# heathsc/bs_call

Measured on AMD Instinct MI355X. Metric: genome positions called/sec, higher is better.
Workload: dtype f64

## Files before the change

bs_call_amd/csrc/prepdev.hip:

```cpp
#include <hip/hip_runtime.h>
#include <stdint.h>

#include "../../include/bscall_amd.h"

#define FLT_QUAL 63u

struct bsc_prep_plan {
  uint64_t src;
  uint64_t ms;
  uint32_t rl0;
  uint32_t w0, wl;
  uint32_t nm;
  uint32_t mark_l, mark_r;
  uint32_t out_len;
  uint32_t present;
  uint32_t trim_l, trim_r;
};

struct bsc_prep_desc {
  uint64_t srcw;
  uint32_t pk;
  int32_t pc;
};
#define PD_PRESENT 1u
#define PD_EDITED 2u
#define PD_SLOW 8u

#define PREP_CNT_WORDS 8u
#define PREP_CNT_SLOTS 64u
#define PE_ORI 1u
#define PE_READ 2u
#define PE_LIST 4u
#define PE_SOFT_POS 6u
#define PE_SOFT_ILL 7u
#define PE_INDEL 8u
#define PE_CAP 9u
#define PE_PROF_CAP 10u
#define PE_PROF_RANGE 11u

struct prep_rd {
  uint32_t w0, wl;
};
__device__ static __forceinline__ void d_left_trim(prep_rd &r, uint32_t l) {
  if (l > 0) {
    if (l >= r.wl) r.wl = 0;
    else {
      r.w0 += l;
      r.wl -= l;
    }
  }
}
__device__ static __forceinline__ void d_right_trim(prep_rd &r, uint32_t l) {
  if (l > 0) {
    if (l >= r.wl) r.wl = 0;
    else r.wl -= l;
  }
}

__device__ static __forceinline__ uint32_t d_qual(const uint8_t *sp, uint32_t i, uint32_t rl0, uint32_t mark_l, uint32_t mark_r) {
  return (i < mark_l || i >= rl0 - mark_r) ? FLT_QUAL : (uint32_t)sp[i] >> 2;
}

__device__ static __forceinline__ uint32_t d_ld32(const uint8_t *p);
__device__ static uint32_t d_mean_qual(const uint8_t *sp, const prep_rd &r, uint32_t rl0, uint32_t mark_l, uint32_t mark_r) {
  const uint32_t lo = r.w0 > mark_l ? r.w0 : mark_l;
  const uint32_t e0 = r.w0 + r.wl, e1 = rl0 - mark_r;
  const uint32_t hi = e0 < e1 ? e0 : e1;
  uint32_t tot = 0, n = 0, i = lo;
#define MQ_DWORD(w_)                                                                                                                   \
  {                                                                                                                                    \
    const uint32_t q = ((w_) >> 2) & 0x3f3f3f3fu;                                                                                      \
    const uint32_t nz = ((q ^ 0x3f3f3f3fu) + 0x7f7f7f7fu) & 0x80808080u;  \
    n += (uint32_t)__popc(nz);                                                                                                         \
    tot = __builtin_amdgcn_sad_u8(q & ((nz >> 7) * 0xffu), 0u, tot);                                       \
  }
  for (; i + 16u <= hi; i += 16u) {
    uint4 v;
    __builtin_memcpy(&v, sp + i, 16);
    MQ_DWORD(v.x) MQ_DWORD(v.y) MQ_DWORD(v.z) MQ_DWORD(v.w)
  }
  for (; i + 4u <= hi; i += 4u) MQ_DWORD(d_ld32(sp + i))
#undef MQ_DWORD
  for (; i < hi; i++) {
    const uint32_t q = (uint32_t)sp[i] >> 2;
    if (q != FLT_QUAL) {
      tot += q;
      n++;
    }
  }
  return n > 0 ? tot / n : 0;
}

__global__ __launch_bounds__(256) void bsc_prep_plan_kernel(const bsc_raw_template *__restrict__ raw, uint32_t nr, const uint8_t *__restrict__ seq,
                                                            uint64_t seq_bytes, const bsc_misms *__restrict__ misms_in, uint64_t n_misms_in,
                                                            bsc_prep_params par, bsc_misms *__restrict__ ms_work,
                                                            bsc_prep_plan *__restrict__ plan, bsc_prep_desc *__restrict__ desc,
                                                            unsigned long long *__restrict__ out_len,
                                                            bsc_template *__restrict__ tpl_out, unsigned long long *__restrict__ cnt,
                                                            uint32_t *__restrict__ max_pos1) {
  const uint32_t ti = blockIdx.x * 256u + threadIdx.x;
  unsigned long long n_clip = 0, n_overlap = 0;
  uint32_t err = 0;
  if (ti < nr) {
    const bsc_raw_template t = raw[ti];
    bsc_prep_plan P[2];
    prep_rd rd[2];
    uint32_t nm[2];
    bsc_misms *ms[2];
    bool edited[2] = {false, false};
    uint32_t pos[2] = {t.pos[0], t.pos[1]};
    if (t.orientation > 1) err = PE_ORI;
#pragma unroll
    for (int k = 0; k < 2 && !err; k++) {
      if (t.len[k] && (t.off[k] > seq_bytes || t.len[k] > seq_bytes - t.off[k])) err = PE_READ + (uint32_t)k;
      else if (t.n_misms[k] && (t.misms_off[k] > n_misms_in || t.n_misms[k] > n_misms_in - t.misms_off[k])) err = PE_LIST + (uint32_t)k;
    }
    if (!err) {
      const int msk = t.orientation == 0 ? 0 : 1;
#pragma unroll
      for (int k = 0; k < 2; k++) {
        const int side = k ^ msk;
        const uint32_t rl = t.len[k];
        const int32_t lt = side ? par.left_trim[1] : par.left_trim[0], rt = side ? par.right_trim[1] : par.right_trim[0];
        P[k].src = t.off[k];
        P[k].ms = t.misms_off[k];
        P[k].rl0 = rl;
        P[k].mark_l = lt > 0 ? ((uint32_t)lt < rl ? (uint32_t)lt : rl) : 0u;
        P[k].mark_r = rt > 0 ? ((uint32_t)rt < rl ? (uint32_t)rt : rl) : 0u;
        P[k].present = rl != 0;
        P[k].trim_l = P[k].trim_r = 0;
        rd[k].w0 = 0;
        rd[k].wl = rl;
        nm[k] = t.n_misms[k];
        ms[k] = ms_work + t.misms_off[k];
        for (uint32_t z = 0; z < nm[k]; z++) ms[k][z] = misms_in[t.misms_off[k] + z];
      }
#pragma unroll
      for (int k = 0; k < 2 && !err; k++) {
        const uint32_t rl = rd[k].wl;
        if (rl == 0) continue;
        int nclip = 0;
        uint32_t adj = 0;
        const uint32_t n0 = nm[k];
        for (uint32_t z = 0; z < n0; z++) {
          bsc_misms *m = ms[k] + z;
          if (m->type == BSC_MISMS_SOFT) {
            if (z && z != n0 - 1) { err = PE_SOFT_POS; break; }
            nclip++;
            if (!m->position) {
              if (m->size >= rl) { err = PE_SOFT_ILL; break; }
              adj = m->size;
              n_clip += adj;
              P[k].trim_l = adj;
              d_left_trim(rd[k], adj);
            } else {
              if (m->position + m->size != rl) { err = PE_SOFT_ILL; break; }
              d_right_trim(rd[k], m->size);
              P[k].trim_r = m->size;
              n_clip += m->size;
            }
          } else if (nclip) {
            m->position -= adj;
            ms[k][z - (uint32_t)nclip] = *m;
          }
        }
        if (nclip) nm[k] -= (uint32_t)nclip;
      }
    }
    if (!err) {
      const uint32_t rdl[2] = {rd[0].wl, rd[1].wl};
      if (rdl[0] > 0 && rdl[1] > 0) {
        int rev;
        int32_t overlap;
        if (pos[0] <= pos[1]) {
          overlap = (int32_t)(t.reference_span[0] - pos[1] + pos[0]);
          rev = 0;
        } else {
          overlap = (int32_t)(t.reference_span[1] + pos[1] - pos[0]);
          rev = 1;
        }
        if (pos[0] + t.reference_span[0] >= pos[1]) {
          int tr;
          if (t.reference_span[0] > t.reference_span[1]) tr = 1;
          else if (t.reference_span[0] < t.reference_span[1]) tr = 0;
          else
            tr = d_mean_qual(seq + P[0].src, rd[0], P[0].rl0, P[0].mark_l, P[0].mark_r) <=
                         d_mean_qual(seq + P[1].src, rd[1], P[1].rl0, P[1].mark_l, P[1].mark_r)
                     ? 0
                     : 1;
          const int right = (rev && tr) || !(rev || tr);
          if (!right) {
            if (tr) pos[1] += (uint32_t)overlap;
            else pos[0] += (uint32_t)overlap;
          }
          bsc_misms *mm = tr ? ms[1] : ms[0];
          prep_rd rdt = tr ? rd[1] : rd[0];
          const uint32_t rdl_t = tr ? rdl[1] : rdl[0], span_t = tr ? t.reference_span[1] : t.reference_span[0];
          uint32_t num = tr ? nm[1] : nm[0];
          if (!num) {
            if (right) d_right_trim(rdt, (uint32_t)overlap);
            else d_left_trim(rdt, (uint32_t)overlap);
          } else {
            int trimmed = 0;
            if (right) {
              const uint32_t xx = span_t - (uint32_t)overlap;
              int64_t adj = 0;
              for (uint32_t z = 0; z < num; z++) {
                bsc_misms *m = mm + z;
                if ((int64_t)m->position + adj >= (int64_t)xx) {
                  const int64_t trim = (int64_t)rdl_t - xx + adj;
                  d_right_trim(rdt, (uint32_t)trim);
                  num = z;
                  trimmed = 1;
                  break;
                }
                if (m->type == BSC_MISMS_INS) {
                  if ((int64_t)m->position + adj + m->size >= (int64_t)xx) {
                    const int64_t trim = (int64_t)rdl_t - m->position;
                    m->size = (uint32_t)((int64_t)xx - ((int64_t)m->position + adj));
                    d_right_trim(rdt, (uint32_t)trim);
                    num = z + 1;
                    trimmed = 1;
                  }
                  adj += m->size;
                } else if (m->type == BSC_MISMS_DEL) adj -= m->size;
              }
              if (!trimmed) d_right_trim(rdt, (uint32_t)overlap);
            } else {
              const uint32_t xx = (uint32_t)overlap;
              int64_t adj = 0;
              uint32_t z;
              for (z = 0; z < num; z++) {
                bsc_misms *m = mm + z;
                if ((int64_t)m->position + adj >= (int64_t)xx) {
                  const uint32_t trim = (uint32_t)((int64_t)overlap - adj);
                  d_left_trim(rdt, trim);
                  trimmed = 1;
                  if (z) {
                    for (uint32_t z1 = z; z1 < num; z1++) {
                      mm[z1].position -= trim;
                      const bsc_misms a = mm[z1], b = mm[z1 - z];
                      mm[z1 - z] = a;
                      mm[z1] = b;
                    }
                    num -= z;
                  } else {
                    for (uint32_t z1 = 0; z1 < num; z1++) mm[z1].position -= trim;
                  }
                  break;
                }
                if (m->type == BSC_MISMS_INS) {
                  if ((int64_t)m->position + adj + m->size >= (int64_t)xx) {
                    m->size = (uint32_t)((int64_t)m->position + m->size + adj - xx);
                    const uint32_t trim = m->position;
                    d_left_trim(rdt, trim);
                    trimmed = 1;
                    const uint32_t z2 = m->size ? z : z + 1;
                    for (uint32_t z1 = z2; z1 < num; z1++) {
                      mm[z1].position -= trim;
                      if (z2) {
                        const bsc_misms a = mm[z1], b = mm[z1 - z2];
                        mm[z1 - z2] = a;
                        mm[z1] = b;
                      }
                    }
                    num -= z2;
                    break;
                  }
                  adj += m->size;
                } else if (m->type == BSC_MISMS_DEL) adj -= m->size;
              }
              if (!trimmed) {
                d_left_trim(rdt, (uint32_t)((int64_t)overlap - adj));
                num = 0;
              }
            }
          }
          if (tr) {
            nm[1] = num;
            rd[1] = rdt;
          } else {
            nm[0] = num;
            rd[0] = rdt;
          }
          n_overlap += (rdl[0] - rd[0].wl) + (rdl[1] - rd[1].wl);
          const uint32_t cut = tr ? rdl[1] - rd[1].wl : rdl[0] - rd[0].wl;
          if (right) {
            if (tr) P[1].trim_r += cut;
            else P[0].trim_r += cut;
          } else {
            if (tr) P[1].trim_l += cut;
            else P[0].trim_l += cut;
          }
        }
      }
#pragma unroll
      for (int k = 0; k < 2 && !err; k++) {
        const uint32_t rl = rd[k].wl;
        uint32_t adj = 0;
        for (uint32_t z = 0; z < nm[k]; z++) {
          bsc_misms *m = ms[k] + z;
          const uint32_t ix1 = m->position + adj;
          edited[k] |= m->type == BSC_MISMS_INS || m->type == BSC_MISMS_DEL;
          if (m->type == BSC_MISMS_INS) {
            if (ix1 > rl + adj) { err = PE_INDEL; break; }
            adj += m->size;
          } else if (m->type == BSC_MISMS_DEL) {
            if ((uint64_t)ix1 + m->size > (uint64_t)rl + adj) { err = PE_INDEL; break; }
            adj -= m->size;
          }
          m->position = ix1;
        }
        P[k].w0 = rd[k].w0;
        P[k].wl = rl;
        P[k].nm = nm[k];
        P[k].out_len = rl + adj;
      }
    }
    if (err) {
#pragma unroll
      for (int k = 0; k < 2; k++) {
        P[k].src = P[k].ms = 0;
        P[k].rl0 = P[k].w0 = P[k].wl = P[k].nm = P[k].mark_l = P[k].mark_r = P[k].out_len = P[k].present = P[k].trim_l = P[k].trim_r = 0;
      }
      atomicMin(&cnt[0], ((unsigned long long)ti << 8) | err);
      n_clip = n_overlap = 0;
    }
#pragma unroll
    for (int k = 0; k < 2; k++) {
      bsc_prep_desc d;
      const uint32_t ol = P[k].out_len;
      d.srcw = P[k].src + P[k].w0;
      const uint32_t ml = P[k].mark_l > P[k].w0 ? (P[k].mark_l - P[k].w0 < ol ? P[k].mark_l - P[k].w0 : ol) : 0u;
      const uint32_t keep = P[k].rl0 - P[k].mark_r;
      const uint32_t hr = keep > P[k].w0 ? (keep - P[k].w0 < ol ? keep - P[k].w0 : ol) : 0u;
      const bool ed = edited[k] && !err;
      const bool slow = ol != 0 && (ed || hr < ol || ol < 4u || ol >= 0xfffffu || ml >= 256u);
      d.pk = (ol < 0xfffffu ? ol : 0xfffffu) | ((ml & 0xffu) << 20) |
             (((P[k].present ? PD_PRESENT : 0u) | (ed ? PD_EDITED : 0u) | (slow ? PD_SLOW : 0u)) << 28);
      d.pc = k ? (int32_t)(P[k].wl + P[k].trim_r) - 1 : (int32_t)P[k].trim_l;
      desc[2u * ti + (uint32_t)k] = d;
      if (slow) plan[2u * ti + (uint32_t)k] = P[k];
    }
    if (max_pos1) {
      int32_t max_pos = 0;
#pragma unroll
      for (int k = 0; k < 2; k++)
        if (P[k].present) {
          const int32_t mpos = k ? (int32_t)(P[k].wl + P[k].trim_r) - 1 : (int32_t)(P[k].trim_l + P[k].wl);
          if (mpos > max_pos) max_pos = mpos;
        }
      max_pos1[ti] = err ? 0u : (uint32_t)max_pos + 1u;
    }
    out_len[2u * ti] = P[0].out_len;
    out_len[2u * ti + 1u] = P[1].out_len;
    bsc_template o;
    o.pos[0] = pos[0];
    o.pos[1] = pos[1];
    o.len[0] = P[0].out_len;
    o.len[1] = P[1].out_len;
    o.off[0] = o.off[1] = 0;
    o.mapq[0] = t.mapq[0];
    o.mapq[1] = t.mapq[1];
    o.orientation = t.orientation;
    o.bs_strand = t.bs_strand;
    o.flags = 0;
    tpl_out[ti] = o;
  }
  for (int o = 32; o > 0; o >>= 1) {
    n_clip += __shfl_xor(n_clip, o);
    n_overlap += __shfl_xor(n_overlap, o);
  }
  if ((threadIdx.x & 63u) == 0) {
    unsigned long long *slot = cnt + PREP_CNT_WORDS + (blockIdx.x & (PREP_CNT_SLOTS - 1u)) * 8u;
    if (n_clip) atomicAdd(&slot[0], n_clip);
    if (n_overlap) atomicAdd(&slot[1], n_overlap);
  }
}

__device__ static __forceinline__ uint32_t d_marked(const uint8_t *sp, uint32_t i, uint32_t rl0, uint32_t mark_l, uint32_t mark_r) {
  const bool in_r = i >= rl0 - mark_r;
  const uint32_t b = sp[(in_r && 2u * i > rl0 - 1u) ? rl0 - 1u - i : i];
  return (i < mark_l || in_r) ? (b & 3u) | (FLT_QUAL << 2) : (uint32_t)sp[i];
}

struct bsc_prep_prof {
  const uint8_t *ref;
  uint32_t x, n_ref, cap, used0;
  const uint32_t *used_scan;
  unsigned long long *table;
};
__device__ static const uint8_t PROF_REF[64] = {
    0, 0, 0, 0, 0, 0, 0, 0, 0, 0, 0, 8, 0, 0, 0, 0, 0, 4, 4, 0, 4, 0, 0, 0, 0, 0, 0, 8, 0, 0, 0, 0,
    0, 0, 0, 8, 0, 0, 0, 0, 0, 0, 0, 0, 0, 0, 0, 0, 0, 0, 0, 0, 0, 0, 0, 0, 0, 0, 0, 0, 0, 0, 0, 0};
__device__ static __forceinline__ uint32_t d_profile_base(uint32_t bs_strand, uint32_t c) {
  const uint32_t q = c >> 2;
  if (q < 20u  || q >= FLT_QUAL || bs_strand > 2u) return 0u;
  return ((bs_strand == 0 ? 0x7A6Bu : (bs_strand == 1 ? 0x5A4Bu : 0x7869u)) >> (4u * (c & 3u))) & 15u;
}

#define PREP_WAVES 4
#define PREP_BATCH 4u
#define PROF_LDS 512u

__device__ static __forceinline__ void d_prof_base(const bsc_prep_prof &F, uint32_t *s_prof, uint32_t strand, uint32_t used_t, int64_t v,
                                                   int32_t orig, uint32_t byte) {
  const uint32_t xx = d_profile_base(strand, byte);
  if (xx && v + 1 < (int64_t)F.n_ref) {
    const uint32_t ra = v >= 1 ? F.ref[v - 1] : 0u, rb = v >= 0 ? F.ref[v] : 0u, rc = F.ref[v + 1];
    const uint32_t m_before = PROF_REF[((ra << 3) | rb) & 63u], m_after = PROF_REF[((rb << 3) | rc) & 63u];
    if ((((xx & m_after) | ((xx & m_before) >> 1)) >> 2) & 1u) {
      const uint32_t ix = (uint32_t)(orig + 1);
      if (ix < used_t && ix < F.cap) {
        if (ix < PROF_LDS) atomicAdd(&s_prof[(xx & 3u) * PROF_LDS + ix], 1u);
        else atomicAdd(&F.table[(uint64_t)ix * 4u + (xx & 3u)], 1ull);
      }
    }
  }
}

__device__ static __forceinline__ uint32_t d_bcast(uint32_t v, uint32_t l) { return (uint32_t)__builtin_amdgcn_readlane((int)v, (int)l); }
__device__ static __forceinline__ unsigned long long d_bcast64(unsigned long long v, uint32_t l) {
  return (unsigned long long)d_bcast((uint32_t)v, l) | ((unsigned long long)d_bcast((uint32_t)(v >> 32), l) << 32);
}
__device__ static __forceinline__ uint32_t d_ld32(const uint8_t *p) {
  uint32_t v;
  __builtin_memcpy(&v, p, 4);
  return v;
}
__device__ static __forceinline__ void d_st32(uint8_t *p, uint32_t v) { __builtin_memcpy(p, &v, 4); }

struct prep_slow_ret {
  uint32_t c63, cge;
  uint32_t walked;
};

__device__ static __forceinline__ uint32_t prep_slow_src(const bsc_prep_plan &P, const bsc_misms *__restrict__ ms, bool edited, uint32_t j, bool &pad) {
  uint32_t s = j;
  pad = false;
  if (edited) {
    for (uint32_t z = P.nm; z-- > 0;) {
      const bsc_misms m = ms[z];
      if (m.type == BSC_MISMS_INS) {
        if (s >= m.position) {
          if (s - m.position < m.size) {
            pad = true;
            break;
          }
          s -= m.size;
        }
      } else if (m.type == BSC_MISMS_DEL) {
        if (s >= m.position) s += m.size;
      }
    }
  }
  return s;
}

__device__ __noinline__ static prep_slow_ret prep_slow_read(const bsc_prep_plan *__restrict__ plan_r, uint32_t flags, uint8_t *__restrict__ dp,
                                                            const uint8_t *__restrict__ seq, const bsc_misms *__restrict__ ms_work, uint32_t mq) {
  const unsigned lane = threadIdx.x & 63u;
  prep_slow_ret r = {0u, 0u, 0u};
  const bsc_prep_plan P = *plan_r;
  const uint8_t *const sp = seq + P.src;
  const bool edited = (flags & PD_EDITED) != 0;
  if (edited) {
    for (uint32_t s0 = 0; s0 < P.wl; s0 += 64u) {
      const uint32_t s = s0 + lane;
      if (s < P.wl) {
        const uint32_t q = d_marked(sp, P.w0 + s, P.rl0, P.mark_l, P.mark_r) >> 2;
        r.c63 += q == FLT_QUAL;
        r.cge += q >= mq;
      }
    }
  }
  const bsc_misms *const ms = ms_work + P.ms;
  bool walked = false;
  for (uint32_t j0 = 0; j0 < P.out_len; j0 += 64u) {
    const uint32_t j = j0 + lane;
    if (j < P.out_len) {
      bool pad;
      const uint32_t s = prep_slow_src(P, ms, edited, j, pad);
      const uint32_t byte = pad ? 0u : d_marked(sp, P.w0 + s, P.rl0, P.mark_l, P.mark_r);
      const uint32_t q = byte >> 2;
      if (!edited) {
        r.c63 += q == FLT_QUAL;
        r.cge += q >= mq;
      }
      walked |= q != 0 && q != FLT_QUAL;
      dp[j] = (uint8_t)byte;
    }
  }
  r.walked = __any(walked) ? 1u : 0u;
  return r;
}

__global__ __launch_bounds__(64 * PREP_WAVES) void bsc_prep_copy_kernel(const bsc_prep_plan *__restrict__ plan,
                                                                        const bsc_prep_desc *__restrict__ desc, uint32_t nr,
                                                                        const uint8_t *__restrict__ seq, const bsc_misms *__restrict__ ms_work,
                                                                        const unsigned long long *__restrict__ out_off, int32_t min_qual,
                                                                        bsc_template *__restrict__ tpl_out, uint8_t *__restrict__ seq_out,
                                                                        uint64_t seq_out_cap, unsigned long long *__restrict__ cnt) {
  const unsigned lane = threadIdx.x & 63u, lane4 = lane * 4u;
  const uint32_t wave = (uint32_t)__builtin_amdgcn_readfirstlane((int)(blockIdx.x * PREP_WAVES + (threadIdx.x >> 6)));
  const uint32_t n_waves = gridDim.x * PREP_WAVES;
  const uint32_t mq = min_qual < 0 ? 0u : (min_qual > 64 ? 64u : (uint32_t)min_qual), mq4 = mq * 0x01010101u;
  unsigned long long l_total = 0, l_bases = 0;
  uint32_t c63 = 0, cge = 0, l_reads = 0;
  const uint32_t n_reads2 = 2u * nr, n_groups = (n_reads2 + 63u) / 64u;
  for (uint32_t g = wave; g < n_groups; g += n_waves) {
    const uint32_t g0 = g * 64u, n = n_reads2 - g0 < 64u ? n_reads2 - g0 : 64u;
    const uint32_t ri = g0 + (lane < n ? lane : 0u), my_ti = ri >> 1, my_k = ri & 1u;
    bsc_prep_desc L = desc[ri];
    const unsigned long long l_off = out_off[ri];
    if (lane >= n) L.pk = 0;
    if (lane < n) {
      const uint32_t fl = L.pk >> 28;
      uint32_t ol = L.pk & 0xfffffu, wl = ol;
      if (fl & PD_SLOW) {
        ol = plan[ri].out_len;
        wl = plan[ri].wl;
      }
      tpl_out[my_ti].off[my_k] = l_off;
      if (l_off > seq_out_cap || seq_out_cap - l_off < ol) {
        atomicMin(&cnt[0], ((unsigned long long)my_ti << 8) | PE_CAP);
        L.pk &= 0xf0000000u;
      }
      l_total += (fl & PD_EDITED) ? wl : ol;
      if (fl & PD_PRESENT) {
        l_reads++;
        l_bases += wl;
      }
    }
    enum : uint32_t { KIND_LEAN = 1u, KIND_FAST = 2u, KIND_SLOW = 3u };
    const uint32_t my_len = L.pk & 0xfffffu, my_ml = (L.pk >> 20) & 0xffu;
    const uint32_t my_kind = my_len == 0 ? 0u : ((L.pk >> 28) & PD_SLOW ? KIND_SLOW : ((my_len <= 256u && my_ml == 0) ? KIND_LEAN : KIND_FAST));
    const uint32_t l_ctl = (L.pk & 0x0fffffffu) | (my_kind << 28) | (((L.pk >> 28) & PD_EDITED) ? 1u << 30 : 0u);
    const bool my_fetch = my_kind == KIND_LEAN || my_kind == KIND_FAST;
    const unsigned long long l_src = my_fetch ? (unsigned long long)(seq + L.srcw) - (unsigned long long)desc : 0ull;
    unsigned long long walked_mask = 0;
    const unsigned long long obase = d_bcast64(l_off, 0);
    const unsigned long long m_w0 = __ballot(my_kind == KIND_LEAN && my_len >= 16u && my_len <= 128u);
    const unsigned long long sbase = m_w0 ? d_bcast64(L.srcw, (uint32_t)__builtin_ctzll(m_w0)) : 0ull;
    const unsigned long long orel = l_off - obase, srel = L.srcw - sbase;
    const bool my_wide = my_kind == KIND_LEAN && my_len >= 16u && my_len <= 128u && orel < (1ull << 24) && srel < (1ull << 31);
    const uint32_t w_a = my_wide ? my_len | ((uint32_t)orel << 8) : 0u, w_s = my_wide ? (uint32_t)srel : 0u;
    const uint32_t l16 = (lane & 7u) * 16u, sub = lane & 56u;
    const uint8_t *const sp_w = seq + sbase;
    uint8_t *const dp_w = seq_out + obase;
    uint32_t walk_bits = 0;
    constexpr uint32_t RW = 2u;
    auto fetch8 = [&](uint32_t i0, uint4(&vv)[RW]) {
#pragma unroll
      for (uint32_t i = 0; i < RW; i++) {
        const int src = (int)(sub | ((i0 + i) & 7u));
        const uint32_t len = (uint32_t)__shfl((int)w_a, src) & 0xffu, so = (uint32_t)__shfl((int)w_s, src);
        const uint32_t last = len ? len - 16u : 0u;
        __builtin_memcpy(&vv[i], sp_w + (so + (l16 < last ? l16 : last)), 16);
      }
    };
    auto process8 = [&](const uint32_t i0, const uint4(&v)[RW]) {
#pragma unroll
      for (uint32_t i = 0; i < RW; i++) {
        const uint32_t l = i0 + i;
        const int src = (int)(sub | l);
        const uint32_t a_ = (uint32_t)__shfl((int)w_a, src), len = a_ & 0xffu;
        const bool act = l16 < len;
        const uint32_t o = l16 < len - 16u ? l16 : len - 16u, dup = act ? l16 - o : 16u;
        const uint32_t w4[4] = {v[i].x, v[i].y, v[i].z, v[i].w};
        uint32_t any = 0;
#pragma unroll
        for (uint32_t d = 0; d < 4u; d++) {
          const uint32_t ge = (((0x83828180u + 0x04040404u * d) - dup * 0x01010101u) >> 7) & 0x01010101u;
          const uint32_t wc = w4[d] & (ge * 0xffu);
          const uint32_t qh = ((wc >> 2) & 0x3f3f3f3fu) | 0x80808080u;
          const uint32_t q1 = qh + 0x01010101u;
          c63 += (uint32_t)__popc(q1 & 0x40404040u);
          cge += (uint32_t)__popc((qh - mq4) & 0x80808080u);
          any |= q1 & 0x3e3e3e3eu;
        }
        if (any) walk_bits |= 1u << l;
        if (act) __builtin_memcpy(dp_w + ((a_ >> 8) + o), &v[i], 16);
      }
    };
    auto one = [&](const uint32_t l) {
      const uint32_t k = l & 1u;
      const uint32_t ctl = d_bcast(l_ctl, l), kind = (ctl >> 28) & 3u, len = ctl & 0xfffffu;
      uint8_t *const dp = seq_out + d_bcast64(l_off, l);
      if (kind == KIND_SLOW) {
        const prep_slow_ret r = prep_slow_read(plan + g0 + l, (ctl >> 30) & 1u ? PD_EDITED : 0u, dp, seq, ms_work, mq);
        c63 += r.c63;
        cge += r.cge;
        if (k == 0 && r.walked) walked_mask |= 1ull << l;
        return;
      }
      const uint32_t ml = (ctl >> 20) & 0xffu;
      bool walked = false;
      for (uint32_t base = 0; base < len; base += 256u) {
        const uint32_t nominal = base + lane4;
        const bool act = nominal < len;
        const uint32_t o = nominal < len - 4u ? nominal : len - 4u;
        uint32_t w = act ? d_ld32((const uint8_t *)desc + d_bcast64(l_src, l) + o) : 0u;
        if (ml + 3u > base) {
          const uint32_t nmk = act && ml > o ? (ml - o < 4u ? ml - o : 4u) : 0u;
          const uint32_t mm = nmk >= 4u ? 0xffffffffu : (1u << (8u * nmk)) - 1u;
          w = (w & ~mm) | (((w & 0x03030303u) | 0xfcfcfcfcu) & mm);
        }
        const uint32_t wc = act ? w >> (8u * (nominal - o)) : 0u;
        const uint32_t qh = ((wc >> 2) & 0x3f3f3f3fu) | 0x80808080u;
        const uint32_t q1 = qh + 0x01010101u;
        c63 += (uint32_t)__popc(q1 & 0x40404040u);
        cge += (uint32_t)__popc((qh - mq4) & 0x80808080u);
        if (k == 0) walked |= __any((q1 & 0x3e3e3e3eu) != 0u) != 0;
        if (act) d_st32(dp + o, w);
      }
      if (k == 0 && walked) walked_mask |= 1ull << l;
    };
    if (__ballot(my_wide)) {
      uint4 va[RW], vb[RW];
      fetch8(0, va);
#pragma unroll
      for (uint32_t i0 = 0; i0 < 8u; i0 += 2u * RW) {
        fetch8(i0 + RW, vb);
        process8(i0, va);
        fetch8(i0 + 2u * RW, va);
        process8(i0 + RW, vb);
      }
      walk_bits |= (uint32_t)__shfl_xor((int)walk_bits, 1);
      walk_bits |= (uint32_t)__shfl_xor((int)walk_bits, 2);
      walk_bits |= (uint32_t)__shfl_xor((int)walk_bits, 4);
      walked_mask |= __ballot((walk_bits >> (lane & 7u)) & 1u);
    }
    for (unsigned long long rest = __ballot(my_kind != 0u && !my_wide); rest; rest &= rest - 1ull) one((uint32_t)__builtin_ctzll(rest));
    if (lane < n && my_k == 0) tpl_out[my_ti].flags = BSC_TPL_WALK_KNOWN | (((walked_mask >> lane) & 1ull) ? BSC_TPL_WALKED0 : 0u);
  }
  unsigned long long w[5] = {l_total, c63, cge, l_reads, l_bases};
  for (int i = 0; i < 5; i++)
    for (int o = 32; o > 0; o >>= 1) w[i] += __shfl_xor(w[i], o);
  if (mq == 0) w[2] = w[0];
  if (lane == 0) {
    const unsigned long long low = w[0] - w[2] - (mq > FLT_QUAL ? w[1] : 0ull), none = w[0] - w[1] - low;
    if (none) atomicAdd(&cnt[3], none);
    if (w[1]) atomicAdd(&cnt[4], w[1]);
    if (low) atomicAdd(&cnt[5], low);
    if (w[3]) atomicAdd(&cnt[6], w[3]);
    if (w[4]) atomicAdd(&cnt[7], w[4]);
  }
}

__global__ __launch_bounds__(256) void bsc_prep_refmask_kernel(const uint8_t *__restrict__ ref, uint32_t n_ref, uint8_t *__restrict__ mask) {
  const uint64_t i = ((uint64_t)blockIdx.x * 256u + threadIdx.x) * 4u;
  if (i >= (uint64_t)n_ref + 24u) return;
  uint32_t m = 0;
  if (i >= 12u && i - 8u + 7u <= n_ref) {
    const uint64_t v = i - 8u;
    const uint32_t lo = d_ld32(ref + v - 1u) & 0x07070707u, hi = d_ld32(ref + v + 3u) & 0x07070707u;
    const uint32_t r_at = __builtin_amdgcn_alignbyte(hi, lo, 1u), r_next = __builtin_amdgcn_alignbyte(hi, lo, 2u);
#define PROF_NE(x, c) ((((x) ^ ((c) * 0x01010101u)) + 0x7f7f7f7fu) & 0x80808080u)
    const uint32_t over_c = ~PROF_NE(r_at, 2u) & PROF_NE(r_next, 0u) & PROF_NE(r_next, 3u) & 0x80808080u;
    const uint32_t over_g = ~PROF_NE(r_at, 3u) & PROF_NE(lo, 0u) & PROF_NE(lo, 2u) & 0x80808080u;
#undef PROF_NE
    m = (over_c >> 5) | (over_g >> 4);
  } else {
    for (uint32_t t = 0; t < 4u; t++) {
      const uint64_t it = i + t;
      if (it >= 8u && it - 8u + 1u < n_ref) {
        const uint64_t v = it - 8u;
        const uint32_t ra = v >= 1 ? ref[v - 1] : 0u, rb = ref[v], rc = ref[v + 1];
        m |= ((PROF_REF[((rb << 3) | rc) & 63u] & 4u) | (PROF_REF[((ra << 3) | rb) & 63u] & 8u)) << (8u * t);
      }
    }
  }
  __builtin_memcpy(mask + i, &m, 4);
}

__global__ __launch_bounds__(64 * PREP_WAVES) void bsc_prep_profile_kernel(const bsc_prep_plan *__restrict__ plan, const bsc_prep_desc *__restrict__ desc,
                                                                           uint32_t nr, const bsc_misms *__restrict__ ms_work,
                                                                           const unsigned long long *__restrict__ out_off,
                                                                           const bsc_template *__restrict__ tpl_out, const uint8_t *__restrict__ seq_out,
                                                                           uint64_t seq_out_cap, unsigned long long *__restrict__ cnt,
                                                                           const uint8_t *__restrict__ mask, const bsc_prep_prof F) {
  __shared__ uint32_t s_prof[PROF_LDS * 4u];
  for (unsigned i = threadIdx.x; i < PROF_LDS * 4u; i += 64 * PREP_WAVES) s_prof[i] = 0;
  __syncthreads();
  const unsigned lane = threadIdx.x & 63u;
  const uint32_t wave = (uint32_t)__builtin_amdgcn_readfirstlane((int)(blockIdx.x * PREP_WAVES + (threadIdx.x >> 6)));
  const uint32_t n_waves = gridDim.x * PREP_WAVES;
  const uint32_t n_reads2 = 2u * nr, n_groups = (n_reads2 + 63u) / 64u;
  uint32_t acc[4][2] = {{0u, 0u}, {0u, 0u}, {0u, 0u}, {0u, 0u}};
  uint32_t acc_n = 0;
  bool acc_quarter = true;
  auto flush = [&]() {
    const uint32_t p0 = 8u * (acc_quarter ? (lane & 15u) : (lane & 31u));
#pragma unroll
    for (uint32_t b = 0; b < 4u; b++) {
      const uint32_t col = (0x63u >> (2u * b)) & 3u;
#pragma unroll
      for (uint32_t t = 0; t < 8u; t++) {
        const uint32_t c = (acc[b][t >> 2] >> (8u * (t & 3u))) & 0xffu;
        if (c) atomicAdd(&s_prof[col * PROF_LDS + p0 + t + 1u], c);
      }
      acc[b][0] = acc[b][1] = 0u;
    }
    acc_n = 0;
  };
  for (uint32_t g = wave; g < n_groups; g += n_waves) {
    const uint32_t g0 = g * 64u, n = n_reads2 - g0 < 64u ? n_reads2 - g0 : 64u;
    const uint32_t ri = g0 + (lane < n ? lane : 0u), my_ti = ri >> 1, my_k = ri & 1u;
    const bsc_prep_desc L = desc[ri];
    const unsigned long long l_off = out_off[ri];
    const uint32_t us_prev = my_ti ? F.used_scan[my_ti - 1u] : 0u, us_mine = F.used_scan[my_ti];
    const uint32_t t_strand = tpl_out[my_ti].bs_strand, t_pos = tpl_out[my_ti].pos[my_k];
    uint32_t c1 = 0, kind = 0, l_used = 0, l_strand = 0, l_ol = 0, top = 0;
    if (lane < n) {
      const uint32_t fl = L.pk >> 28;
      uint32_t ol = L.pk & 0xfffffu;
      if (fl & PD_SLOW) ol = plan[ri].out_len;
      const bool fits = !(l_off > seq_out_cap || seq_out_cap - l_off < ol);
      if ((fl & PD_PRESENT) && ol != 0 && fits) {
        const uint32_t before = my_ti ? (us_prev > F.used0 ? us_prev : F.used0) : F.used0;
        l_used = us_mine > before ? us_mine : before;
        if (l_used > before && (unsigned long long)l_used + 1ull > F.cap) atomicMin(&cnt[0], ((unsigned long long)my_ti << 8) | PE_PROF_CAP);
        l_strand = t_strand;
        const uint32_t pos = t_pos;
        l_ol = ol;
        const bool in_ref = pos >= F.x && (uint64_t)pos - F.x + ol + 1u <= F.n_ref;
        if (!in_ref) atomicMin(&cnt[0], ((unsigned long long)my_ti << 8) | PE_PROF_RANGE);
        if (in_ref && l_strand <= 2u) {
          const uint32_t lim = l_used < F.cap ? l_used : F.cap;
          const int32_t pc = L.pc;
          top = my_k ? (uint32_t)(pc < 0 ? 0 : pc) : (uint32_t)pc + ol - 1u;
          const bool regs = !(fl & PD_SLOW) && l_strand != 0u && ol <= 256u && pc >= 0 && pc < 512 && top < 256u && top + 1u < lim && l_off >= 8u &&
                            seq_out_cap - l_off - ol >= 8u;
          kind = regs ? 1u : 2u;
          c1 = pos > F.x ? pos - F.x + 1u : 0u;
        }
      }
    }
    unsigned long long m_regs = __ballot(kind == 1u);
    if (m_regs) {
      const uint32_t first = (uint32_t)__builtin_ctzll(m_regs);
      const unsigned long long obase = d_bcast64(l_off, first);
      const unsigned long long orel = l_off - obase;
      if (kind == 1u && orel >= (1ull << 15)) kind = 2u;
      const uint32_t A1 = kind == 1u ? (c1 + 7u) | (l_strand == 2u ? 1u << 29 : 0u) | (1u << 31) : 0u;
      const uint32_t A2 = kind == 1u ? (l_ol - 1u) | ((uint32_t)L.pc << 8) | ((uint32_t)orel << 17) : 0u;
      const bool quarter = __ballot(kind == 1u && top >= 128u) == 0ull;
      if (quarter != acc_quarter) {
        flush();
        acc_quarter = quarter;
      }
      const uint8_t *const sb = seq_out + obase - 8u;
      const uint32_t h = quarter ? (lane & 15u) : (lane & 31u);
      const int32_t p0 = (int32_t)(8u * h);
      const uint32_t hsel = quarter ? (lane & 48u) : (lane & 32u), rounds = quarter ? 16u : 32u;
      constexpr uint32_t B = 2u;
      struct rnd {
        uint32_t a1;
        unsigned long long w, mw;
        int32_t jc, len8;
      };
      auto ask = [&](uint32_t i, rnd &r) {
        const int src = (int)(hsel | (i & (rounds - 1u)));
        r.a1 = (uint32_t)__shfl((int)A1, src);
        const uint32_t a2 = (uint32_t)__shfl((int)A2, src);
        const int32_t len = (int32_t)(a2 & 0xffu) + 1;
        r.len8 = 8 - len;
        const int32_t pc = (int32_t)((a2 >> 8) & 0x1ffu);
        const int32_t j0 = (i & 1u) ? pc - p0 - 7 : p0 - pc;
        const bool some = (int32_t)r.a1 < 0 && (uint32_t)(j0 + 7) < (uint32_t)(len + 7);
        r.jc = some ? j0 : 0;
        __builtin_memcpy(&r.w, sb + ((a2 >> 17) + (uint32_t)(r.jc + 8)), 8);
        __builtin_memcpy(&r.mw, mask + (some ? (r.a1 & 0x1fffffffu) + (uint32_t)j0 : 0u), 8);
      };
      auto count = [&](uint32_t i, const rnd &r) {
        const int32_t lo = r.jc < 0 ? -r.jc : 0, hi = r.jc + r.len8 > 0 ? r.jc + r.len8 : 0;
        unsigned long long w8 = r.w & (~0ull << (8 * lo)) & (~0ull >> (8 * hi));
        unsigned long long m8 = r.mw;
        if (i & 1u) {
          w8 = __builtin_bswap64(w8);
          m8 = __builtin_bswap64(m8);
        }
        const uint32_t sx = (r.a1 >> 29) & 1u ? 0xffffffffu : 0u;
#pragma unroll
        for (int d = 0; d < 2; d++) {
          const uint32_t w = (uint32_t)(w8 >> (32 * d)), mw = (uint32_t)(m8 >> (32 * d));
          const uint32_t odd = w << 7;
          const uint32_t qf = ((w >> 2) & 0x3f3f3f3fu) | 0x80808080u;
          const uint32_t q_ok = (qf - 20u * 0x01010101u) & ~((qf + 0x01010101u) << 1) & 0x80808080u;
          const uint32_t hb = (((odd & (mw << 5)) | (~odd & (mw << 4))) & q_ok) >> 7;
          const uint32_t wb = w ^ sx;
          const uint32_t t1 = hb & (wb >> 1), t0 = hb ^ t1, t3 = t1 & wb, t2 = t0 & wb;
          acc[3][d] += t3;
          acc[2][d] += t1 ^ t3;
          acc[1][d] += t2;
          acc[0][d] += t0 ^ t2;
        }
      };
      rnd ra[B], rb[B];
#pragma unroll
      for (uint32_t u = 0; u < B; u++) ask(u, ra[u]);
      for (uint32_t i0 = 0; i0 < rounds; i0 += 2u * B) {
        if (acc_n + 2u * B > 255u) flush();
#pragma unroll
        for (uint32_t u = 0; u < B; u++) ask(i0 + B + u, rb[u]);
#pragma unroll
        for (uint32_t u = 0; u < B; u++) count(u, ra[u]);
#pragma unroll
        for (uint32_t u = 0; u < B; u++) ask(i0 + 2u * B + u, ra[u]);
#pragma unroll
        for (uint32_t u = 0; u < B; u++) count(B + u, rb[u]);
        acc_n += 2u * B;
      }
    }
    unsigned long long m_long = __ballot(kind == 2u);
    while (m_long) {
      const uint32_t l = (uint32_t)__builtin_ctzll(m_long);
      m_long &= m_long - 1ull;
      const uint32_t ol = d_bcast(l_ol, l), k = l & 1u, strand = d_bcast(l_strand, l), used_t = d_bcast(l_used, l);
      const int32_t pc = (int32_t)d_bcast((uint32_t)L.pc, l);
      const int64_t v0 = (int64_t)d_bcast(c1, l) - 1;
      const uint8_t *const dp = seq_out + d_bcast64(l_off, l);
      const bool slow = (d_bcast(L.pk, l) >> 28) & PD_SLOW;
      bsc_prep_plan P;
      bool edited = false;
      if (slow) {
        P = plan[g0 + l];
        edited = (d_bcast(L.pk, l) >> 28) & PD_EDITED;
      }
      for (uint32_t jb = 0; jb < ol; jb += 64u) {
        const uint32_t j = jb + lane;
        if (j < ol) {
          bool pad = false;
          const uint32_t s = slow ? prep_slow_src(P, ms_work + P.ms, edited, j, pad) : j;
          if (!pad) d_prof_base(F, s_prof, strand, used_t, v0 + j, k ? pc - (int32_t)s : pc + (int32_t)s, dp[j]);
        }
      }
    }
  }
  flush();
  __syncthreads();
  for (unsigned i = threadIdx.x; i < PROF_LDS * 4u; i += 64 * PREP_WAVES)
    if (s_prof[i] && i % PROF_LDS < F.cap) atomicAdd(&F.table[(uint64_t)(i % PROF_LDS) * 4u + i / PROF_LDS], (unsigned long long)s_prof[i]);
}

extern "C" int bsc_dev_scan_u64(const void *in, void *out, uint32_t n, void *tmp, size_t tmp_bytes, void *stream);

extern "C" size_t bsc_dev_prep_plan_bytes(void) { return sizeof(bsc_prep_plan) + sizeof(bsc_prep_desc); }

extern "C" int bsc_dev_scan_max_u32(const void *in, void *out, uint32_t n, void *tmp, size_t tmp_bytes, void *stream);

extern "C" int bsc_dev_launch_prep(const void *raw, uint32_t nr, const void *seq, uint64_t seq_bytes, const void *misms, uint64_t n_misms,
                                   const bsc_prep_params *par, void *ms_work, void *plan, void *out_len, void *out_off, void *scan_tmp,
                                   size_t scan_tmp_bytes, void *tpl_out, void *seq_out, uint64_t seq_out_cap, void *cnt, int num_cus,
                                   void *stream, const void *prof_ref, uint32_t prof_x, uint32_t prof_n_ref, uint32_t prof_cap,
                                   uint32_t prof_used0, void *prof_table, void *max_pos1, void *used_scan, void *prof_mask) {
  hipStream_t s = (hipStream_t)stream;
  bsc_prep_desc *const desc = (bsc_prep_desc *)((bsc_prep_plan *)plan + 2ull * nr);
  if (!nr) return (int)hipMemsetAsync(out_off, 0, sizeof(unsigned long long), s);
  hipError_t e = hipMemsetAsync((unsigned long long *)out_len + 2ull * nr, 0, sizeof(unsigned long long), s);
  if (e != hipSuccess) return (int)e;
  hipLaunchKernelGGL(bsc_prep_plan_kernel, dim3((nr + 255u) / 256u), dim3(256), 0, s, (const bsc_raw_template *)raw, nr, (const uint8_t *)seq,
                     seq_bytes, (const bsc_misms *)misms, n_misms, *par, (bsc_misms *)ms_work, (bsc_prep_plan *)plan, desc,
                     (unsigned long long *)out_len, (bsc_template *)tpl_out, (unsigned long long *)cnt, prof_ref ? (uint32_t *)max_pos1 : nullptr);
  if ((e = hipGetLastError()) != hipSuccess) return (int)e;
  int rc = bsc_dev_scan_u64(out_len, out_off, 2u * nr + 1u, scan_tmp, scan_tmp_bytes, stream);
  if (rc) return rc;
  bsc_prep_prof F = {nullptr, 0u, 0u, 0u, 0u, nullptr, nullptr};
  if (prof_ref) {
    if ((rc = bsc_dev_scan_max_u32(max_pos1, used_scan, nr, scan_tmp, scan_tmp_bytes, stream))) return rc;
    F.ref = (const uint8_t *)prof_ref;
    F.x = prof_x;
    F.n_ref = prof_n_ref;
    F.cap = prof_cap;
    F.used0 = prof_used0;
    F.used_scan = (const uint32_t *)used_scan;
    F.table = (unsigned long long *)prof_table;
  }
  unsigned g = ((nr + 31u) / 32u + PREP_WAVES - 1u) / PREP_WAVES;
  static int per_cu[2] = {0, 0};
  for (int pv = 0; pv < (prof_ref ? 2 : 1); pv++)
    if (!per_cu[pv]) {
      int nb = 0;
      const hipError_t eo = pv ? hipOccupancyMaxActiveBlocksPerMultiprocessor(&nb, bsc_prep_profile_kernel, 64 * PREP_WAVES, 0)
                               : hipOccupancyMaxActiveBlocksPerMultiprocessor(&nb, bsc_prep_copy_kernel, 64 * PREP_WAVES, 0);
      per_cu[pv] = (eo == hipSuccess && nb > 0) ? nb : 4;
      (void)hipGetLastError();
    }
  unsigned gc = g, gp = g;
  if (gc > (unsigned)num_cus * (unsigned)per_cu[0]) gc = (unsigned)num_cus * (unsigned)per_cu[0];
  hipLaunchKernelGGL(bsc_prep_copy_kernel, dim3(gc), dim3(64 * PREP_WAVES), 0, s, (const bsc_prep_plan *)plan, (const bsc_prep_desc *)desc, nr,
                     (const uint8_t *)seq, (const bsc_misms *)ms_work, (const unsigned long long *)out_off, par->min_qual, (bsc_template *)tpl_out,
                     (uint8_t *)seq_out, seq_out_cap, (unsigned long long *)cnt);
  if ((e = hipGetLastError()) != hipSuccess) return (int)e;
  if (prof_ref) {
    hipLaunchKernelGGL(bsc_prep_refmask_kernel, dim3((unsigned)(((uint64_t)prof_n_ref + 24u + 1023u) / 1024u)), dim3(256), 0, s, (const uint8_t *)prof_ref,
                       prof_n_ref, (uint8_t *)prof_mask);
    if ((e = hipGetLastError()) != hipSuccess) return (int)e;
    if (gp > (unsigned)num_cus * (unsigned)per_cu[1]) gp = (unsigned)num_cus * (unsigned)per_cu[1];
    hipLaunchKernelGGL(bsc_prep_profile_kernel, dim3(gp), dim3(64 * PREP_WAVES), 0, s, (const bsc_prep_plan *)plan, (const bsc_prep_desc *)desc, nr,
                       (const bsc_misms *)ms_work, (const unsigned long long *)out_off, (const bsc_template *)tpl_out, (const uint8_t *)seq_out,
                       seq_out_cap, (unsigned long long *)cnt, (const uint8_t *)prof_mask, F);
  }
  return (int)hipGetLastError();
}
```

Measured before the change: 16.74 billion.

## Stage short lean reads in per-wave LDS image and flush contiguous runs

Instead of each lane writing unaligned 16-byte chunks of short reads straight to global output, the wide path now writes them into a per-wave LDS image. Each contiguous run of wide reads is then copied out with aligned, coalesced stores through the recstream copy helpers. A prefix scan over gap sizes places the non-wide reads' space outside the image, and non-wide reads break runs. The change adds 32KB of LDS per block, which may lower occupancy, and adds wave syncs and an extra copy pass.

```diff
diff --git a/bs_call_amd/csrc/prepdev.hip b/bs_call_amd/csrc/prepdev.hip
--- a/bs_call_amd/csrc/prepdev.hip
+++ b/bs_call_amd/csrc/prepdev.hip
@@ -2,6 +2,7 @@
 #include <stdint.h>
 
 #include "../../include/bscall_amd.h"
+#include "recstream_dev.h"
 
 #define FLT_QUAL 63u
 
@@ -402,6 +403,7 @@
 #define PREP_WAVES 4
 #define PREP_BATCH 4u
 #define PROF_LDS 512u
+#define PREP_IMG 8192u
 
 __device__ static __forceinline__ void d_prof_base(const bsc_prep_prof &F, uint32_t *s_prof, uint32_t strand, uint32_t used_t, int64_t v,
                                                    int32_t orig, uint32_t byte) {
@@ -501,7 +503,9 @@
                                                                         const unsigned long long *__restrict__ out_off, int32_t min_qual,
                                                                         bsc_template *__restrict__ tpl_out, uint8_t *__restrict__ seq_out,
                                                                         uint64_t seq_out_cap, unsigned long long *__restrict__ cnt) {
+  __shared__ __attribute__((aligned(16))) uint8_t s_img[PREP_WAVES][PREP_IMG];
   const unsigned lane = threadIdx.x & 63u, lane4 = lane * 4u;
+  uint8_t *const img = s_img[threadIdx.x >> 6];
   const uint32_t wave = (uint32_t)__builtin_amdgcn_readfirstlane((int)(blockIdx.x * PREP_WAVES + (threadIdx.x >> 6)));
   const uint32_t n_waves = gridDim.x * PREP_WAVES;
   const uint32_t mq = min_qual < 0 ? 0u : (min_qual > 64 ? 64u : (uint32_t)min_qual), mq4 = mq * 0x01010101u;
@@ -514,6 +518,7 @@
     bsc_prep_desc L = desc[ri];
     const unsigned long long l_off = out_off[ri];
     if (lane >= n) L.pk = 0;
+    uint32_t t_ol = 0;
     if (lane < n) {
       const uint32_t fl = L.pk >> 28;
       uint32_t ol = L.pk & 0xfffffu, wl = ol;
@@ -521,6 +526,7 @@
         ol = plan[ri].out_len;
         wl = plan[ri].wl;
       }
+      t_ol = ol;
       tpl_out[my_ti].off[my_k] = l_off;
       if (l_off > seq_out_cap || seq_out_cap - l_off < ol) {
         atomicMin(&cnt[0], ((unsigned long long)my_ti << 8) | PE_CAP);
@@ -542,12 +548,26 @@
     const unsigned long long obase = d_bcast64(l_off, 0);
     const unsigned long long m_w0 = __ballot(my_kind == KIND_LEAN && my_len >= 16u && my_len <= 128u);
     const unsigned long long sbase = m_w0 ? d_bcast64(L.srcw, (uint32_t)__builtin_ctzll(m_w0)) : 0ull;
-    const unsigned long long orel = l_off - obase, srel = L.srcw - sbase;
-    const bool my_wide = my_kind == KIND_LEAN && my_len >= 16u && my_len <= 128u && orel < (1ull << 24) && srel < (1ull << 31);
-    const uint32_t w_a = my_wide ? my_len | ((uint32_t)orel << 8) : 0u, w_s = my_wide ? (uint32_t)srel : 0u;
+    const unsigned long long srel = L.srcw - sbase;
+    const bool my_w0 = my_kind == KIND_LEAN && my_len >= 16u && my_len <= 128u && srel < (1ull << 31);
+    const uint32_t img_ph = (uint32_t)((unsigned long long)(seq_out + obase) & 15ull);
+    const uint32_t my_gap = my_w0 ? 0u : t_ol & ~15u;
+    uint32_t gap_before = 0;
+    if (__ballot(my_gap != 0u)) {
+      uint32_t inc = my_gap;
+#pragma unroll
+      for (int d = 1; d < 64; d <<= 1) {
+        const uint32_t up = (uint32_t)__shfl_up((int)inc, d);
+        if (lane >= (unsigned)d) inc += up;
+      }
+      gap_before = inc - my_gap;
+    }
+    const uint32_t my_io = img_ph + (uint32_t)(l_off - obase) - gap_before;
+    const bool my_wide = my_w0 && my_io + my_len <= PREP_IMG;
+    const unsigned long long m_brk = __ballot(!my_wide && t_ol != 0u);
+    const uint32_t w_a = my_wide ? my_len | (my_io << 8) : 0u, w_s = my_wide ? (uint32_t)srel : 0u;
     const uint32_t l16 = (lane & 7u) * 16u, sub = lane & 56u;
     const uint8_t *const sp_w = seq + sbase;
-    uint8_t *const dp_w = seq_out + obase;
     uint32_t walk_bits = 0;
     constexpr uint32_t RW = 2u;
     auto fetch8 = [&](uint32_t i0, uint4(&vv)[RW]) {
@@ -580,7 +600,7 @@
           any |= q1 & 0x3e3e3e3eu;
         }
         if (any) walk_bits |= 1u << l;
-        if (act) __builtin_memcpy(dp_w + ((a_ >> 8) + o), &v[i], 16);
+        if (act) __builtin_memcpy(img + ((a_ >> 8) + o), &v[i], 16);
       }
     };
     auto one = [&](const uint32_t l) {
@@ -630,6 +650,17 @@
       walk_bits |= (uint32_t)__shfl_xor((int)walk_bits, 2);
       walk_bits |= (uint32_t)__shfl_xor((int)walk_bits, 4);
       walked_mask |= __ballot((walk_bits >> (lane & 7u)) & 1u);
+      rs_wave_sync();
+      for (unsigned long long mw = __ballot(my_wide); mw;) {
+        const uint32_t a = (uint32_t)__builtin_ctzll(mw);
+        const unsigned long long brk = m_brk & (~0ull << a);
+        const unsigned long long run = brk ? mw & ((1ull << (uint32_t)__builtin_ctzll(brk)) - 1ull) : mw;
+        const uint32_t b = 63u - (uint32_t)__builtin_clzll(run);
+        const uint32_t i0 = d_bcast(my_io, a), i1 = d_bcast(my_io + my_len, b), piece0 = i0 & ~15u;
+        rs_copy_out(img + piece0, seq_out + (d_bcast64(l_off, a) - (i0 - piece0)), lane, rs_copy_ranges(i0 - piece0, i1 - i0));
+        mw &= ~run;
+      }
+      rs_wave_sync();
     }
     for (unsigned long long rest = __ballot(my_kind != 0u && !my_wide); rest; rest &= rest - 1ull) one((uint32_t)__builtin_ctzll(rest));
     if (lane < n && my_k == 0) tpl_out[my_ti].flags = BSC_TPL_WALK_KNOWN | (((walked_mask >> lane) & 1ull) ? BSC_TPL_WALKED0 : 0u);
```

Result: no change. 16.66 billion (-0.5%).
